# NeuroDiffGym/neurodiffeq

Hardware: NVIDIA B200
Metric: collocation-points/sec (residual+grad) (higher is better)
Workload: dtype f32

## Files before the change

experiments/tcgen05_probe/probe_wgrad.cu:

```cuda
#include <cstdio>
#include <cstdlib>
#include <cstdint>
#include <cmath>
#include <vector>
#include <cuda_runtime.h>
#include <cuda_bf16.h>

#define CK(x) do { cudaError_t e_ = (x); if (e_ != cudaSuccess) { printf("CUDA error %s at %s:%d\n", cudaGetErrorString(e_), __FILE__, __LINE__); return 2; } } while (0)

__device__ __forceinline__ uint32_t smem_u32(const void* p) { return (uint32_t)__cvta_generic_to_shared(p); }

__device__ __forceinline__ uint64_t make_desc(uint32_t saddr, uint32_t lbo_enc, uint32_t sbo_enc) {
    uint64_t d = 0;
    d |= (uint64_t)((saddr & 0x3FFFF) >> 4);
    d |= (uint64_t)(lbo_enc & 0x3FFF) << 16;
    d |= (uint64_t)(sbo_enc & 0x3FFF) << 32;
    d |= (uint64_t)1 << 46;
    d |= (uint64_t)2 << 61;
    return d;
}

constexpr int ROWS = 256, H = 64, IMG = ROWS * 128;

__global__ void __launch_bounds__(128, 1) probe_kernel(const uint8_t* __restrict__ z_img, const uint8_t* __restrict__ a_img,
// ... 41 lines not shown
            smem_u32(mbar))
        : "memory");
    asm volatile("tcgen05.fence::after_thread_sync;" ::: "memory");

    const uint32_t lane_addr = taddr + ((uint32_t)(warp * 32) << 16);
    const int tl = warp * 32 + lane;
#pragma unroll
    for (int c0 = 0; c0 < H; c0 += 16) {
        uint32_t v[16];
        asm volatile(
            "tcgen05.ld.sync.aligned.32x32b.x16.b32 {%0,%1,%2,%3,%4,%5,%6,%7,%8,%9,%10,%11,%12,%13,%14,%15}, [%16];\n"
            : "=r"(v[0]), "=r"(v[1]), "=r"(v[2]), "=r"(v[3]), "=r"(v[4]), "=r"(v[5]), "=r"(v[6]), "=r"(v[7]), "=r"(v[8]),
              "=r"(v[9]), "=r"(v[10]), "=r"(v[11]), "=r"(v[12]), "=r"(v[13]), "=r"(v[14]), "=r"(v[15])
            : "r"(lane_addr + c0));
        asm volatile("tcgen05.wait::ld.sync.aligned;" ::: "memory");
#pragma unroll
        for (int j = 0; j < 16; ++j) d_out[tl * H + c0 + j] = __uint_as_float(v[j]);
    }
    asm volatile("tcgen05.fence::before_thread_sync;" ::: "memory");
    __syncthreads();
    if (warp == 0) asm volatile("tcgen05.dealloc.cta_group::1.sync.aligned.b32 %0, 64;" ::"r"(taddr));
}

static inline size_t sw128_offset(int r, int u) {
    const int b = u * 2;
    return (size_t)(r >> 3) * 1024 + (size_t)(r & 7) * 128 + (size_t)(((b >> 4) ^ (r & 7)) << 4) + (b & 15);
}

int main(int argc, char** argv) {
    const uint32_t lbo = argc > 1 ? atoi(argv[1]) : 0, sbo = argc > 2 ? atoi(argv[2]) : 64;
    const int M = argc > 3 ? atoi(argv[3]) : 64, k_adv = argc > 4 ? atoi(argv[4]) : 2048;
    std::vector<float> Z0(ROWS * H), Z1(ROWS * H), A(ROWS * H);
    srand(3);
    for (auto& x : Z0) x = (float)(rand() % 7 - 3);
    for (auto& x : Z1) x = (float)(rand() % 5 - 2);
    for (auto& x : A) x = (float)(rand() % 7 - 3);
    std::vector<uint8_t> zi(2 * IMG, 0), ai(IMG, 0);
    for (int r = 0; r < ROWS; ++r)
        for (int u = 0; u < H; ++u) {
            *reinterpret_cast<__nv_bfloat16*>(&zi[sw128_offset(r, u)]) = __float2bfloat16(Z0[r * H + u]);
            *reinterpret_cast<__nv_bfloat16*>(&zi[IMG + sw128_offset(r, u)]) = __float2bfloat16(Z1[r * H + u]);
            *reinterpret_cast<__nv_bfloat16*>(&ai[sw128_offset(r, u)]) = __float2bfloat16(A[r * H + u]);
        }
    std::vector<double> ref(128 * H, 0.0);
    for (int m = 0; m < 128; ++m)
        for (int n = 0; n < H; ++n) {
            double s = 0;
            for (int r = 0; r < ROWS; ++r) s += (double)(m < 64 ? Z0[r * H + m] : Z1[r * H + m - 64]) * (double)A[r * H + n];
            ref[m * H + n] = s;
        }
    uint8_t *dz, *da;
    float* dd;
// ... 25 lines not shown
```

neurodiffeq_b200/csrc/pinnjet_k2tc2.cuh:

```cuda
#pragma once
#include "pinnjet_tc.cuh"

namespace pj {

constexpr int K2T_THREADS = TC_NT + 64;
#ifndef PJ_WG_FIRST
#define PJ_WG_FIRST 0
#endif

template <int N1, int N2, int WL>
__device__ __forceinline__ void act_from_record(int act, const float (&z)[1 + N1 + N2], float (&a)[1 + N1 + N2], const float* w) {
    float a0, s1, s2;
    if (act == PJ_ACT_TANH) {
        a0 = z[0];
        s1 = fmaf(-a0, a0, 1.0f);
        s2 = -2.0f * a0 * s1;
    } else {
        sincosf(z[0], &a0, &s1);
        s2 = -a0;
    }
    a[0] = a0;
#pragma unroll
    for (int f = 0; f < N1; ++f) a[1 + f] = s1 * z[1 + f];
    if constexpr (WL > 0) {
        float q = 0.0f;
#pragma unroll
        for (int d = 0; d < WL; ++d) q = fmaf(w[d] * z[1 + d], z[1 + d], q);
        a[1 + N1] = fmaf(s2, q, s1 * z[1 + N1]);
    } else {
#pragma unroll
        for (int s = 0; s < N2; ++s) a[1 + N1 + s] = fmaf(s2 * z[1 + s], z[1 + s], s1 * z[1 + N1 + s]);
// ... 15 lines not shown
    unsigned char* wimg = smem + pl.k2_ring;
    float* stage = reinterpret_cast<float*>(smem + pl.k2_zb);
    float* wlo_s = reinterpret_cast<float*>(smem + pl.k2_small);
    float* tinfo = wlo_s + sp.n_nets * PJ_MAX_NETS * TC_H;
    float* recbuf = reinterpret_cast<float*>(smem + pl.k2_ybar);
    float* sgrad = reinterpret_cast<float*>(smem + pl.k2_sgrad);
    uint64_t* wfull = reinterpret_cast<uint64_t*>(smem + pl.k2_misc);
    uint64_t* z_ready = wfull + 1;
    uint64_t* a_ready = wfull + 2;
    uint64_t* adj_done = wfull + 3;
    uint64_t* wg_done = wfull + 4;
    uint64_t* rec_full = wfull + 5;
    uint64_t* rec_empty = wfull + 6;
    uint64_t* ti_full = wfull + 7;
    uint64_t* ti_empty = wfull + 9;
    uint32_t* tmem_slot = reinterpret_cast<uint32_t*>(wfull + 11);

    const int tid = threadIdx.x, warp = tid >> 5, lane = tid & 31;
    const int n_tiles = pl.n_tiles1;
    const int my_tiles = (n_tiles > (int)blockIdx.x) ? (n_tiles - 1 - (int)blockIdx.x) / (int)gridDim.x + 1 : 0;
    float* gpart = A.gpart + (size_t)blockIdx.x * sp.n_theta;
    int n_hh = 0;
    for (int n = 0; n < sp.n_nets; ++n) n_hh += sp.net[n].n_linear - 2;
    const int tmem_cols = 64 * (1 + n_hh) <= 128 ? 128 : (64 * (1 + n_hh) <= 256 ? 256 : 512);

    pdl_launch_dependents();
    if (tid == 0) {
#ifdef PJ_TIMING
        *reinterpret_cast<unsigned long long*>(tmem_slot + 2) = clock64();
#endif
        mbar_init(wfull, 1);
        mbar_init(z_ready, TC_NCW);
        mbar_init(a_ready, TC_NCW);
        mbar_init(adj_done, 1);
        mbar_init(wg_done, 1);
        mbar_init(rec_full, 1);
        mbar_init(rec_empty, TC_NCW);
        for (int b = 0; b < 2; ++b) {
            mbar_init(&ti_full[b], 1);
            mbar_init(&ti_empty[b], TC_NCW);
        }
        fence_barrier_init();
    }
    if (warp == 0) {
        if (tmem_cols == 128)
            asm volatile("tcgen05.alloc.cta_group::1.sync.aligned.shared::cta.b32 [%0], 128;" ::"r"(smem_u32(tmem_slot)));
        else if (tmem_cols == 256)
            asm volatile("tcgen05.alloc.cta_group::1.sync.aligned.shared::cta.b32 [%0], 256;" ::"r"(smem_u32(tmem_slot)));
        else
            asm volatile("tcgen05.alloc.cta_group::1.sync.aligned.shared::cta.b32 [%0], 512;" ::"r"(smem_u32(tmem_slot)));
        asm volatile("tcgen05.relinquish_alloc_permit.cta_group::1.sync.aligned;");
    }
    for (int i = tid; i < 4 * pl.sgrad_floats; i += K2T_THREADS) sgrad[i] = 0.0f;
    if constexpr (G::CP != C)
        for (int i = tid; i < 2 * 3 * TC_AIMG / 16; i += K2T_THREADS) reinterpret_cast<uint4*>(zimg)[i] = make_uint4(0, 0, 0, 0);
    pdl_wait();
    for (int i = tid; i < sp.n_nets * PJ_MAX_NETS * TC_H; i += K2T_THREADS) {
        const int n = i / (PJ_MAX_NETS * TC_H), r = i - n * (PJ_MAX_NETS * TC_H);
        wlo_s[i] = r < sp.net[n].width[sp.net[n].n_linear] * TC_H ? __ldg(A.pack + pl.s_wlo[n] + r) : 0.0f;
    }
    for (long long i = tid; i < sp.n_theta; i += K2T_THREADS) gpart[i] = 0.0f;
    fence_proxy_async();
    tc_fence_before();
    __syncthreads();
    tc_fence_after();
    const uint32_t tmem_base = *tmem_slot;
#ifdef PJ_TIMING
    const unsigned long long t0_ = *reinterpret_cast<volatile unsigned long long*>(tmem_slot + 2);
#endif

    if (warp == TC_NCW) {
        TC_TRACE(tr, A.dbg, 250, 120, t0_, blockIdx.x == 0 && lane == 0)
        if (lane == 0) {
            if (n_hh > 0) {
                mbar_arrive_expect_tx(wfull, (uint32_t)n_hh * 3u * TC_WIMG);
                int slot = 0;
                for (int n = 0; n < sp.n_nets; ++n)
                    for (int l = 1; l < sp.net[n].n_linear - 1; ++l, ++slot)
                        tma_bulk_g2s(wimg + (size_t)slot * 3 * TC_WIMG, A.pack + pl.b_wimg[n][l], 3 * TC_WIMG, wfull);
            } else {
                mbar_arrive(wfull);
            }
        }
        mbar_wait(wfull, 0);
        constexpr uint32_t IDESC_ADJ = tc_idesc(128, TC_H, false, true), IDESC_WG = tc_idesc(64, TC_H, true, true);
        const uint64_t dz = umma_desc_sw128(smem_u32(zimg)), da = umma_desc_sw128(smem_u32(aimg));
        uint32_t phz = 0, pha = 0;
#pragma unroll 1
        for (int iter = 0; iter < my_tiles; ++iter) {
            int slot0 = 0;
#pragma unroll 1
            for (int n = 0; n < sp.n_nets; ++n) {
                const int L = sp.net[n].n_linear - 1;
#pragma unroll 1
                for (int h = L; h >= 2; --h) {
                    const int slot = slot0 + (h - 2);
                    mbar_wait(z_ready, phz);
                    phz ^= 1u;
                    tc_fence_after();
                    TC_MARK(tr, 1 | (h << 5))
                    if (lane == 0) {
                        tc_mma_split6<TC_H / 16, TC_AIMG, 32, TC_WIMG, 2048>(
                            tmem_base, dz, umma_desc_sw128(smem_u32(wimg + (size_t)slot * 3 * TC_WIMG)), IDESC_ADJ, false);
                        tc_commit(adj_done);
                    }
                    __syncwarp();
                    TC_MARK(tr, 2 | (h << 5))
                    mbar_wait(a_ready, pha);
                    pha ^= 1u;
                    tc_fence_after();
                    TC_MARK(tr, 3 | (h << 5))
                    if (lane == 0) {
                        tc_mma_split6<TC_ROWS / 16, TC_AIMG, 2048, TC_AIMG, 2048, PJ_WG_FIRST>(tmem_base + 64u + (uint32_t)slot * 64u, dz, da,
                                                                                               IDESC_WG, iter > 0);
                        tc_commit(wg_done);
                    }
                    __syncwarp();
                    TC_MARK(tr, 4 | (h << 5))
                }
                slot0 += L - 1;
            }
        }
        return;
    }

    if (warp == TC_NCW + 1) {
        uint32_t ph = 0;
        bool first = true;
        const int NW = sp.n_nets * WL, ti_rows = sp.n_yrows + NW + sp.n_coords;
        auto stage_tile_info = [&](int it) {
            if (it >= 2) mbar_wait(&ti_empty[it & 1], (uint32_t)(((it >> 1) - 1) & 1));
            const long long t = (long long)blockIdx.x + (long long)it * gridDim.x;
            float* dst = tinfo + (size_t)(it & 1) * ti_rows * TP;
            for (int e = lane; e < ti_rows * TP; e += 32) {
                const int row = e / TP, pt = e - row * TP;
                float v;
                if (row < sp.n_yrows) v = __ldg(A.seeds + t * ((long long)sp.n_yrows * TP) + e);
                else if (row < sp.n_yrows + NW) v = __ldg(A.wts + t * ((long long)NW * TP) + (e - sp.n_yrows * TP));
                else v = __ldg(A.coords[row - sp.n_yrows - NW] + min(t * TP + pt, A.N - 1));
                dst[e] = v;
            }
            __syncwarp();
            if (lane == 0) mbar_arrive(&ti_full[it & 1]);
        };
        if (my_tiles > 0) stage_tile_info(0);
#pragma unroll 1
        for (int iter = 0; iter < my_tiles; ++iter) {
            const long long tile = (long long)blockIdx.x + (long long)iter * gridDim.x;
            int lidx0 = 0;
#pragma unroll 1
            for (int n = 0; n < sp.n_nets; ++n) {
                const int L = sp.net[n].n_linear - 1;
#pragma unroll 1
                for (int h = L; h >= 1; --h) {
                    if (!first) {
                        mbar_wait(rec_empty, ph);
                        ph ^= 1u;
                    }
                    first = false;
                    if (lane == 0) {
                        mbar_arrive_expect_tx(rec_full, REC_BYTES);
                        tma_bulk_g2s(recbuf, A.zj + tile * pl.tc_rec_tile_floats + (long long)(lidx0 + h - 1) * pl.tc_rec_layer_floats,
                                     REC_BYTES, rec_full);
                    }
                    __syncwarp();
                    if (n == sp.n_nets - 1 && h == 1 && iter + 1 < my_tiles) stage_tile_info(iter + 1);
                }
                lidx0 += L;
            }
        }
        return;
    }

    const TcThread<C> th(tid);
    float* sg = sgrad + (size_t)th.q * pl.sgrad_floats;
    const bool adder = (th.pt & 1) == 0;
    const int uadd = th.ubase + (th.pt >> 1);
    uint32_t ph_adj = 0, ph_wg = 0, ph_rec = 0;
    bool wg_pending = false;
    TC_TRACE(tr, A.dbg, 0, 250, t0_, blockIdx.x == 0 && tid == 0)
    float zr[C][UG];
#ifdef PJ_DBG_REC_GLOBAL
    long long dbg_rec_off = 0;
#endif
    auto next_record = [&]() {
        mbar_wait(rec_full, ph_rec);
        ph_rec ^= 1u;
#ifdef PJ_DBG_REC_GLOBAL
        tc_load_record<C>(A.zj + dbg_rec_off + (size_t)tid * G::REC, zr);
#else
        tc_load_record_smem<C>(recbuf + (size_t)tid * G::REC, zr);
#endif
        float chk = 0.0f;
#pragma unroll
        for (int c = 0; c < C; ++c)
#pragma unroll
            for (int k = 0; k < UG; ++k) chk += zr[c][k];
        fence_proxy_async();
        __syncwarp();
        if (lane == 0 && __float_as_uint(chk) != 0xFFFFFFFFu) mbar_arrive(rec_empty);
    };

#pragma unroll 1
    for (int iter = 0; iter < my_tiles; ++iter) {
        const int NW = sp.n_nets * WL;
        const float* ti = tinfo + (size_t)(iter & 1) * (sp.n_yrows + NW + sp.n_coords) * TP + th.p;
        mbar_wait(&ti_full[iter & 1], (uint32_t)((iter >> 1) & 1));

#pragma unroll 1
        for (int n = 0; n < sp.n_nets; ++n) {
            const PjNet& net = sp.net[n];
            const int L = net.n_linear - 1;
            const int act_kind = net.act;
            const int n_out = net.width[net.n_linear];
            TC_MARK(tr, 1)
            float wq[WLN];
#pragma unroll
            for (int d = 0; d < WLN; ++d) wq[d] = WL > 0 ? ti[(sp.n_yrows + n * WL + d) * TP] : 0.0f;
            float yb_[PJ_MAX_NETS][C];
            {
                const float* sd = ti + net.yrow0 * TP;
#pragma unroll
                for (int o = 0; o < PJ_MAX_NETS; ++o)
#pragma unroll
                    for (int c = 0; c < C; ++c) yb_[o][c] = o < n_out ? sd[(o * C + c) * TP] : 0.0f;
            }
#ifdef PJ_DBG_REC_GLOBAL
            int dbg_l0 = 0;
            for (int m = 0; m < n; ++m) dbg_l0 += sp.net[m].n_linear - 1;
            dbg_rec_off = tile * pl.tc_rec_tile_floats + (long long)(dbg_l0 + L - 1) * pl.tc_rec_layer_floats;
#endif
            next_record();
            TC_MARK(tr, 2)

            float zb[C][UG];
            {
                const float* wlo = wlo_s + n * PJ_MAX_NETS * TC_H;
                float gwl[PJ_MAX_NETS][UG], gbv[UG];
#pragma unroll
                for (int k = 0; k < UG; ++k) {
                    const int u = th.ubase + k;
                    float z[C], ab[C], a[C], zbk[C];
#pragma unroll
                    for (int c = 0; c < C; ++c) {
                        z[c] = zr[c][k];
                        ab[c] = 0.0f;
                    }
#pragma unroll
                    for (int o = 0; o < PJ_MAX_NETS; ++o)
                        if (o < n_out) {
                            const float w = wlo[o * TC_H + u];
#pragma unroll
                            for (int c = 0; c < C; ++c) ab[c] = fmaf(w, yb_[o][c], ab[c]);
                        }
// ... 12 lines not shown
                {
                    const float s = tc_reduce_points<C>(gbv, th.pt);
                    if (adder) sg[pl.g_b[n][L - 1] + uadd] += s;
                }
#pragma unroll
                for (int o = 0; o < PJ_MAX_NETS; ++o)
                    if (o < n_out) {
                        const float s = tc_reduce_points<C>(gwl[o], th.pt);
                        if (adder) sg[pl.g_wl[n] + o * TC_H + uadd] += s;
                    }
                if (th.j == 0) {
#pragma unroll
                    for (int o = 0; o < PJ_MAX_NETS; ++o)
                        if (o < n_out) {
                            const float s = warp_sum(th.ug == 0 ? yb_[o][0] : 0.0f);
                            if (lane == 0) sg[pl.g_bout[n] + o] += s;
                        }
                }
            }
            TC_MARK(tr, 3)

            if (L >= 2) {
                if (wg_pending) {
                    mbar_wait(wg_done, ph_wg);
                    ph_wg ^= 1u;
                    wg_pending = false;
                }
                tc_store_rows<C>(zimg, TC_AIMG, th, zb);
                tc_publish(z_ready, th.lane);
            }
            TC_MARK(tr, 4)
#pragma unroll 1
            for (int h = L; h >= 2; --h) {
#ifdef PJ_DBG_REC_GLOBAL
                dbg_rec_off -= pl.tc_rec_layer_floats;
#endif
                next_record();
                {
                    float av[C][UG];
#pragma unroll
                    for (int k = 0; k < UG; ++k) {
                        float z[C], a[C];
#pragma unroll
                        for (int c = 0; c < C; ++c) z[c] = zr[c][k];
                        act_from_record<N1, N2, WL>(act_kind, z, a, wq);
#pragma unroll
                        for (int c = 0; c < C; ++c) av[c][k] = a[c];
                    }
                    tc_store_rows<C>(aimg, TC_AIMG, th, av);
                }
                tc_publish(a_ready, th.lane);
                TC_MARK(tr, 5 | (h << 5))

                mbar_wait(adj_done, ph_adj);
                ph_adj ^= 1u;
                tc_fence_after();
                TC_MARK(tr, 6 | (h << 5))
                float ab[C][UG];
                tc_load_owner<C>(tmem_base, stage, th, ab);
                TC_MARK(tr, 7 | (h << 5))
                float gbv[UG];
#pragma unroll
                for (int k = 0; k < UG; ++k) {
                    float z[C], abk[C], a[C], zbk[C];
#pragma unroll
                    for (int c = 0; c < C; ++c) {
                        z[c] = zr[c][k];
                        abk[c] = ab[c][k];
                    }
                    act_backward<N1, N2, WL>(act_kind, z, abk, a, zbk, wq);
#pragma unroll
                    for (int c = 0; c < C; ++c) zb[c][k] = zbk[c];
                    gbv[k] = zbk[0];
                }
                {
                    const float s = tc_reduce_points<C>(gbv, th.pt);
                    if (adder) sg[pl.g_b[n][h - 2] + uadd] += s;
                }
                TC_MARK(tr, 8 | (h << 5))
                wg_pending = true;
                if (h > 2) {
                    mbar_wait(wg_done, ph_wg);
                    ph_wg ^= 1u;
                    wg_pending = false;
                    TC_MARK(tr, 9 | (h << 5))
                    tc_store_rows<C>(zimg, TC_AIMG, th, zb);
                    tc_publish(z_ready, th.lane);
                    TC_MARK(tr, 10 | (h << 5))
                }
            }

            {
#pragma unroll
                for (int i = 0; i < PJ_MAX_COORDS; ++i)
                    if (i < net.n_in) {
                        const int ci = net.in_coord[i];
                        const float x = ti[(sp.n_yrows + NW + ci) * TP];
                        float v[UG];
#pragma unroll
                        for (int k = 0; k < UG; ++k) {
                            float s = zb[0][k] * x;
#pragma unroll
                            for (int f = 0; f < N1; ++f) s = fmaf(zb[1 + f][k], sp.dir[f][ci], s);
                            v[k] = s;
                        }
                        const float s = tc_reduce_points<C>(v, th.pt);
                        if (adder) sg[pl.g_w0[n] + uadd * net.n_in + i] += s;
                    }
            }
            TC_MARK(tr, 11)
        }
        __syncwarp();
        if (lane == 0) mbar_arrive(&ti_empty[iter & 1]);
    }
    TC_MARK(tr, 12)
    if (wg_pending) {
        mbar_wait(wg_done, ph_wg);
        ph_wg ^= 1u;
    }
    TC_MARK(tr, 14)

    tc_fence_after();
    {
        const int SG = pl.sgrad_floats;
        int slot = 0;
#pragma unroll 1
        for (int n = 0; n < sp.n_nets; ++n) {
            bar_named(9, TC_NT);
            TC_MARK(tr, 15)
            const PjNet& net = sp.net[n];
            bool shared_w = false;
            for (int m = 0; m < n; ++m) shared_w = shared_w || sp.net[m].w_off[0] == net.w_off[0];
            const int L = net.n_linear - 1;
            const int h1 = net.width[1], hL = net.width[L], n_out = net.width[net.n_linear];
            auto put = [&](long long off, int s_idx) {
                const float v = (sgrad[s_idx] + sgrad[SG + s_idx]) + (sgrad[2 * SG + s_idx] + sgrad[3 * SG + s_idx]);
                if (shared_w) gpart[off] += v; else gpart[off] = v;
            };
#pragma unroll 1
            for (int e = tid; e < h1 * net.n_in; e += TC_NT) put(net.w_off[0] + e, pl.g_w0[n] + e);
#pragma unroll 1
            for (int hl = 0; hl < L; ++hl)
#pragma unroll 1
                for (int e = tid; e < net.width[hl + 1]; e += TC_NT) put(net.b_off[hl] + e, pl.g_b[n][hl] + e);
#pragma unroll 1
            for (int e = tid; e < n_out * hL; e += TC_NT) {
                const int o = e / hL, k = e - o * hL;
                put(net.w_off[L] + e, pl.g_wl[n] + o * TC_H + k);
            }
#pragma unroll 1
            for (int e = tid; e < n_out; e += TC_NT) put(net.b_off[L] + e, pl.g_bout[n] + e);
            TC_MARK(tr, 16)
#pragma unroll 1
            for (int l = 1; l < L; ++l, ++slot) {
                const int width_j = net.width[l + 1], width_k = net.width[l];
                uint32_t v[16];
                const uint32_t addr = tmem_base + 64u + (uint32_t)slot * 64u + (uint32_t)(th.j * 16) + ((uint32_t)(th.q * 32) << 16);
                asm volatile(
                    "tcgen05.ld.sync.aligned.32x32b.x16.b32 "
                    "{%0,%1,%2,%3,%4,%5,%6,%7,%8,%9,%10,%11,%12,%13,%14,%15}, [%16];\n"
                    : "=r"(v[0]), "=r"(v[1]), "=r"(v[2]), "=r"(v[3]), "=r"(v[4]), "=r"(v[5]), "=r"(v[6]), "=r"(v[7]), "=r"(v[8]),
                      "=r"(v[9]), "=r"(v[10]), "=r"(v[11]), "=r"(v[12]), "=r"(v[13]), "=r"(v[14]), "=r"(v[15])
                    : "r"(addr));
                asm volatile("tcgen05.wait::ld.sync.aligned;" ::: "memory");
                const int jr = 16 * th.q + lane, k0 = th.j * 16;
                if (lane < 16 && jr < width_j) {
                    float* gw = gpart + net.w_off[l] + (size_t)jr * width_k + k0;
#pragma unroll
                    for (int i = 0; i < 16; ++i)
                        if (k0 + i < width_k) {
                            if (shared_w) gw[i] += __uint_as_float(v[i]); else gw[i] = __uint_as_float(v[i]);
                        }
                }
            }
        }
    }
    TC_MARK(tr, 13)
    tc_fence_before();
    bar_named(9, TC_NT);
    if (warp == 0) {
        if (tmem_cols == 128)
            asm volatile("tcgen05.dealloc.cta_group::1.sync.aligned.b32 %0, 128;" ::"r"(tmem_base));
        else if (tmem_cols == 256)
            asm volatile("tcgen05.dealloc.cta_group::1.sync.aligned.b32 %0, 256;" ::"r"(tmem_base));
        else
            asm volatile("tcgen05.dealloc.cta_group::1.sync.aligned.b32 %0, 512;" ::"r"(tmem_base));
    }
}

}
```

neurodiffeq_b200/csrc/pinnjet_tc.cuh:

```cuda
#pragma once
#include "pinnjet_common.cuh"

namespace pj {

constexpr int TC_ROWS = 128;
constexpr int TC_H = 64;
constexpr int TC_AIMG = TC_ROWS * 128;
constexpr int TC_WIMG = TC_H * 128;
constexpr int TC_WOUT = 16 * 128;
constexpr int TC_NCW = 16;
constexpr int TC_NT = TC_NCW * 32;
constexpr int TC_STAGE_STRIDE = 20;
constexpr int TC_STAGE_BYTES = TC_NCW * 32 * TC_STAGE_STRIDE * 4;

template <int C>
struct TcGeo {
    static constexpr int CP = C <= 2 ? 2 : (C <= 4 ? 4 : 8);
    static constexpr int TP = TC_ROWS / CP;
    static constexpr int PW = 32 / CP;
    static constexpr int NUG = 32 / PW;
    static constexpr int UG = 16 / NUG;
    static constexpr int REC = C * UG;
};

__device__ __forceinline__ uint64_t umma_desc_sw128(uint32_t saddr) {
    return (uint64_t)((saddr & 0x3FFFF) >> 4) | ((uint64_t)64 << 32) | ((uint64_t)1 << 46) | ((uint64_t)2 << 61);
}
__device__ __forceinline__ uint32_t sw128_off(int row, int chunk16) {
    return (uint32_t)((row >> 3) * 1024 + (row & 7) * 128 + ((chunk16 ^ (row & 7)) << 4));
}
__device__ __forceinline__ uint32_t pack_bf16x2(float lo, float hi) {
    uint32_t r;
    asm("cvt.rn.bf16x2.f32 %0, %1, %2;" : "=r"(r) : "f"(hi), "f"(lo));
    return r;
}
__device__ __forceinline__ float bf16_lo_f32(uint32_t v) { return __uint_as_float(v << 16); }
__device__ __forceinline__ float bf16_hi_f32(uint32_t v) { return __uint_as_float(v & 0xffff0000u); }

__device__ __forceinline__ void split3_bf16(float x0, float x1, uint32_t& t1, uint32_t& t2, uint32_t& t3) {
    t1 = pack_bf16x2(x0, x1);
    const float r0 = x0 - bf16_lo_f32(t1), r1 = x1 - bf16_hi_f32(t1);
    t2 = pack_bf16x2(r0, r1);
    t3 = pack_bf16x2(r0 - bf16_lo_f32(t2), r1 - bf16_hi_f32(t2));
}

__device__ __forceinline__ void bar_named(int id, int nthreads) {
    asm volatile("bar.sync %0, %1;" ::"r"(id), "r"(nthreads) : "memory");
}
__device__ __forceinline__ void tc_fence_before() { asm volatile("tcgen05.fence::before_thread_sync;" ::: "memory"); }
__device__ __forceinline__ void tc_fence_after() { asm volatile("tcgen05.fence::after_thread_sync;" ::: "memory"); }

__host__ __device__ constexpr uint32_t tc_idesc(int M, int N, bool a_mn, bool b_mn) {
    return (1u << 4) | (1u << 7) | (1u << 10) | (a_mn ? (1u << 15) : 0u) | (b_mn ? (1u << 16) : 0u) |
           ((uint32_t)(N >> 3) << 17) | ((uint32_t)(M >> 4) << 24);
}
__device__ __forceinline__ void tc_mma(uint32_t d_tmem, uint64_t da, uint64_t db, uint32_t idesc, uint32_t accumulate) {
    asm volatile(
        "{\n\t.reg .pred p;\n\tsetp.ne.b32 p, %4, 0;\n\t"
        "tcgen05.mma.cta_group::1.kind::f16 [%0], %1, %2, %3, p;\n\t}\n" ::"r"(d_tmem),
        "l"(da), "l"(db), "r"(idesc), "r"(accumulate)
        : "memory");
}
__device__ __forceinline__ void tc_commit(uint64_t* bar) {
    asm volatile("tcgen05.commit.cta_group::1.mbarrier::arrive::one.shared::cluster.b64 [%0];" ::"r"(smem_u32(bar)) : "memory");
}
template <int KSTEPS, uint32_t A_IMG, uint32_t A_KSTEP, uint32_t B_IMG, uint32_t B_KSTEP, int FIRST = 0>
__device__ __forceinline__ void tc_mma_split6(uint32_t d_tmem, uint64_t da0, uint64_t db0, uint32_t idesc, bool accumulate_first) {
#pragma unroll
    for (int pr = FIRST; pr < 6; ++pr)
#pragma unroll
        for (int k = 0; k < KSTEPS; ++k) {
            constexpr int TA[6] = {0, 2, 1, 0, 1, 0}, TB[6] = {2, 0, 1, 1, 0, 0};
            const uint64_t da = da0 + (uint64_t)((TA[pr] * A_IMG + k * A_KSTEP) >> 4);
            const uint64_t db = db0 + (uint64_t)((TB[pr] * B_IMG + k * B_KSTEP) >> 4);
            tc_mma(d_tmem, da, db, idesc, (accumulate_first || pr > FIRST || k) ? 1u : 0u);
        }
}

#ifdef PJ_TIMING
struct TcTrace {
    uint32_t* buf;
    int n, cap;
    unsigned long long t0;
    bool on;
    __device__ __forceinline__ void mark(int tag) {
        if (on && n < cap) buf[n++] = ((uint32_t)tag << 24) | (uint32_t)((clock64() - t0) & 0xFFFFFFull);
    }
};
#define TC_TRACE(name, dbg, base, cap_, t0_, on_) TcTrace name{reinterpret_cast<uint32_t*>(dbg) + (base), 0, cap_, t0_, on_};
#define TC_MARK(name, tag) name.mark(tag);
#else
#define TC_TRACE(name, dbg, base, cap_, t0_, on_)
#define TC_MARK(name, tag)
#endif

template <int C>
struct TcThread {
    using G = TcGeo<C>;
    int warp, lane, q, j, pt, ug;
// ... 29 lines not shown
    constexpr int UG = TcGeo<C>::UG;
#pragma unroll
    for (int c = 0; c < C; ++c) {
        uint32_t t1[UG / 2], t2[UG / 2], t3[UG / 2];
#pragma unroll
        for (int e = 0; e < UG / 2; ++e) split3_bf16(v[c][2 * e], v[c][2 * e + 1], t1[e], t2[e], t3[e]);
        unsigned char* dst = img + t.img_off(c);
        if constexpr (UG == 2) {
            *reinterpret_cast<uint32_t*>(dst) = t1[0];
            *reinterpret_cast<uint32_t*>(dst + img_bytes) = t2[0];
            *reinterpret_cast<uint32_t*>(dst + 2 * img_bytes) = t3[0];
        } else if constexpr (UG == 4) {
            *reinterpret_cast<uint2*>(dst) = make_uint2(t1[0], t1[1]);
            *reinterpret_cast<uint2*>(dst + img_bytes) = make_uint2(t2[0], t2[1]);
            *reinterpret_cast<uint2*>(dst + 2 * img_bytes) = make_uint2(t3[0], t3[1]);
        } else {
            *reinterpret_cast<uint4*>(dst) = make_uint4(t1[0], t1[1], t1[2], t1[3]);
            *reinterpret_cast<uint4*>(dst + img_bytes) = make_uint4(t2[0], t2[1], t2[2], t2[3]);
            *reinterpret_cast<uint4*>(dst + 2 * img_bytes) = make_uint4(t3[0], t3[1], t3[2], t3[3]);
        }
    }
}

template <int C>
__device__ __forceinline__ void tc_load_owner(uint32_t tmem_acc, float* stage, const TcThread<C>& t,
                                              float (&v)[C][TcGeo<C>::UG]) {
    using G = TcGeo<C>;
    constexpr int UG = G::UG;
    float* my_stage = stage + (size_t)t.warp * 32 * TC_STAGE_STRIDE;
    {
        uint32_t r[16];
        const uint32_t addr = tmem_acc + (uint32_t)(t.j * 16) + ((uint32_t)(t.q * 32) << 16);
        asm volatile(
            "tcgen05.ld.sync.aligned.32x32b.x16.b32 "
            "{%0,%1,%2,%3,%4,%5,%6,%7,%8,%9,%10,%11,%12,%13,%14,%15}, [%16];\n"
            : "=r"(r[0]), "=r"(r[1]), "=r"(r[2]), "=r"(r[3]), "=r"(r[4]), "=r"(r[5]), "=r"(r[6]), "=r"(r[7]), "=r"(r[8]),
              "=r"(r[9]), "=r"(r[10]), "=r"(r[11]), "=r"(r[12]), "=r"(r[13]), "=r"(r[14]), "=r"(r[15])
            : "r"(addr));
        asm volatile("tcgen05.wait::ld.sync.aligned;" ::: "memory");
        float* dst = my_stage + t.lane * TC_STAGE_STRIDE;
#pragma unroll
        for (int s = 0; s < 4; ++s)
            *reinterpret_cast<uint4*>(dst + 4 * s) = make_uint4(r[4 * s], r[4 * s + 1], r[4 * s + 2], r[4 * s + 3]);
    }
    __syncwarp();
    const float* src = my_stage + (size_t)(G::CP * t.pt) * TC_STAGE_STRIDE + t.ug * UG;
#pragma unroll
    for (int c = 0; c < C; ++c) {
        if constexpr (UG == 2) {
            const float2 x = *reinterpret_cast<const float2*>(src + c * TC_STAGE_STRIDE);
            v[c][0] = x.x;
            v[c][1] = x.y;
        } else {
#pragma unroll
            for (int s4 = 0; s4 < UG / 4; ++s4) {
                const float4 x = *reinterpret_cast<const float4*>(src + c * TC_STAGE_STRIDE + 4 * s4);
                v[c][4 * s4 + 0] = x.x;
                v[c][4 * s4 + 1] = x.y;
                v[c][4 * s4 + 2] = x.z;
                v[c][4 * s4 + 3] = x.w;
            }
        }
// ... 105 lines not shown
```

Baseline: 155.5 million.

## Stack split-bf16 MMA terms into wider N=128 tcgen05 tiles and TMA-stage tile info

For networks with few hidden layers, the six split-bf16 product terms of the adjoint and weight-gradient GEMMs are grouped into stacked M128xN128 MMAs using an LBO-strided descriptor, with the partial blocks summed when read back from tensor memory. This cuts the number of MMA instructions and makes better use of the tensor core. Tile-info staging moves from a per-lane load loop to TMA bulk copies issued by the MMA warp, prefetched ahead. Gradient zeroing is skipped when every parameter is owned. The change uses more tensor-memory columns and shared scratch, and needs an extra cross-warp reduction step before gradients are written.

```diff
diff --git a/experiments/tcgen05_probe/probe_wgrad.cu b/experiments/tcgen05_probe/probe_wgrad.cu
--- a/experiments/tcgen05_probe/probe_wgrad.cu
+++ b/experiments/tcgen05_probe/probe_wgrad.cu
@@ -87,12 +87,138 @@
     if (warp == 0) asm volatile("tcgen05.dealloc.cta_group::1.sync.aligned.b32 %0, 64;" ::"r"(taddr));
 }
 
+constexpr int TIMG = 128 * 128, WIMG = 64 * 128;
+__global__ void __launch_bounds__(128, 1) stack_kernel(const uint8_t* __restrict__ z_img, const uint8_t* __restrict__ a_img,
+                                                       const uint8_t* __restrict__ w_img, float* __restrict__ d_out) {
+    extern __shared__ __align__(1024) uint8_t smem[];
+    uint8_t* z_s = smem;
+    uint8_t* a_s = smem + 3 * TIMG;
+    uint8_t* w_s = smem + 6 * TIMG;
+    uint64_t* mbar = reinterpret_cast<uint64_t*>(smem + 6 * TIMG + 3 * WIMG);
+    uint32_t* tmem_slot = reinterpret_cast<uint32_t*>(mbar + 1);
+    const int tid = threadIdx.x, warp = tid >> 5, lane = tid & 31;
+    if (tid == 0) {
+        asm volatile("mbarrier.init.shared::cta.b64 [%0], 1;" ::"r"(smem_u32(mbar)));
+        asm volatile("fence.mbarrier_init.release.cluster;" ::: "memory");
+    }
+    if (warp == 0) {
+        asm volatile("tcgen05.alloc.cta_group::1.sync.aligned.shared::cta.b32 [%0], 512;" ::"r"(smem_u32(tmem_slot)));
+        asm volatile("tcgen05.relinquish_alloc_permit.cta_group::1.sync.aligned;");
+    }
+    for (int i = tid; i < 3 * TIMG / 16; i += 128) {
+        reinterpret_cast<uint4*>(z_s)[i] = reinterpret_cast<const uint4*>(z_img)[i];
+        reinterpret_cast<uint4*>(a_s)[i] = reinterpret_cast<const uint4*>(a_img)[i];
+    }
+    for (int i = tid; i < 3 * WIMG / 16; i += 128) reinterpret_cast<uint4*>(w_s)[i] = reinterpret_cast<const uint4*>(w_img)[i];
+    asm volatile("fence.proxy.async.shared::cta;" ::: "memory");
+    asm volatile("tcgen05.fence::before_thread_sync;" ::: "memory");
+    __syncthreads();
+    asm volatile("tcgen05.fence::after_thread_sync;" ::: "memory");
+    const uint32_t taddr = *tmem_slot;
+    if (tid == 0) {
+        auto mma = [](uint32_t d, uint64_t da, uint64_t db, uint32_t idesc, uint32_t acc) {
+            asm volatile(
+                "{\n\t.reg .pred p;\n\tsetp.ne.b32 p, %4, 0;\n\t"
+                "tcgen05.mma.cta_group::1.kind::f16 [%0], %1, %2, %3, p;\n\t}\n" ::"r"(d),
+                "l"(da), "l"(db), "r"(idesc), "r"(acc)
+                : "memory");
+        };
+        auto idesc = [](int M, int N, bool amn, bool bmn) {
+            return (1u << 4) | (1u << 7) | (1u << 10) | (amn ? 1u << 15 : 0u) | (bmn ? 1u << 16 : 0u) | ((uint32_t)(N >> 3) << 17) |
+                   ((uint32_t)(M >> 4) << 24);
+        };
+        const uint32_t za = smem_u32(z_s), aa = smem_u32(a_s), wa = smem_u32(w_s);
+        for (int k = 0; k < 8; ++k)
+            mma(taddr, make_desc(za + k * 2048, TIMG >> 4, 64), make_desc(aa + k * 2048, TIMG >> 4, 64), idesc(128, 128, true, true), k);
+        for (int k = 0; k < 8; ++k)
+            mma(taddr + 128, make_desc(za + k * 2048, 0, 64), make_desc(aa + 2 * TIMG + k * 2048, 0, 64), idesc(64, 64, true, true), k);
+        for (int k = 0; k < 8; ++k)
+            mma(taddr + 128, make_desc(za + 2 * TIMG + k * 2048, 0, 64), make_desc(aa + k * 2048, 0, 64), idesc(64, 64, true, true), 1);
+        for (int k = 0; k < 4; ++k)
+            mma(taddr + 192, make_desc(za + k * 32, 0, 64), make_desc(wa + k * 2048, WIMG >> 4, 64), idesc(128, 128, false, true), k);
+        asm volatile("tcgen05.commit.cta_group::1.mbarrier::arrive::one.shared::cluster.b64 [%0];" ::"r"(smem_u32(mbar)) : "memory");
+    }
+    asm volatile(
+        "{\n.reg .pred P1;\nLAB_WAIT2:\nmbarrier.try_wait.parity.shared::cta.b64 P1, [%0], 0;\n@P1 bra DONE2;\nbra LAB_WAIT2;\nDONE2:\n}\n" ::"r"(
+            smem_u32(mbar))
+        : "memory");
+    asm volatile("tcgen05.fence::after_thread_sync;" ::: "memory");
+    const uint32_t lane_addr = taddr + ((uint32_t)(warp * 32) << 16);
+    const int tl = warp * 32 + lane;
+    for (int c0 = 0; c0 < 320; c0 += 16) {
+        uint32_t v[16];
+        asm volatile(
+            "tcgen05.ld.sync.aligned.32x32b.x16.b32 {%0,%1,%2,%3,%4,%5,%6,%7,%8,%9,%10,%11,%12,%13,%14,%15}, [%16];\n"
+            : "=r"(v[0]), "=r"(v[1]), "=r"(v[2]), "=r"(v[3]), "=r"(v[4]), "=r"(v[5]), "=r"(v[6]), "=r"(v[7]), "=r"(v[8]),
+              "=r"(v[9]), "=r"(v[10]), "=r"(v[11]), "=r"(v[12]), "=r"(v[13]), "=r"(v[14]), "=r"(v[15])
+            : "r"(lane_addr + c0));
+        asm volatile("tcgen05.wait::ld.sync.aligned;" ::: "memory");
+        for (int j = 0; j < 16; ++j) d_out[tl * 320 + c0 + j] = __uint_as_float(v[j]);
+    }
+    asm volatile("tcgen05.fence::before_thread_sync;" ::: "memory");
+    __syncthreads();
+    if (warp == 0) asm volatile("tcgen05.dealloc.cta_group::1.sync.aligned.b32 %0, 512;" ::"r"(taddr));
+}
+
 static inline size_t sw128_offset(int r, int u) {
     const int b = u * 2;
     return (size_t)(r >> 3) * 1024 + (size_t)(r & 7) * 128 + (size_t)(((b >> 4) ^ (r & 7)) << 4) + (b & 15);
 }
 
+static int run_stack() {
+    const int R = 128;
+    std::vector<float> Z[3], A[3], W[3];
+    srand(5);
+    for (int t = 0; t < 3; ++t) {
+        Z[t].resize(R * H); A[t].resize(R * H); W[t].resize(H * H);
+        for (auto& x : Z[t]) x = (float)(rand() % 7 - 3);
+        for (auto& x : A[t]) x = (float)(rand() % 5 - 2);
+        for (auto& x : W[t]) x = (float)(rand() % 7 - 3);
+    }
+    std::vector<uint8_t> zi(3 * TIMG, 0), ai(3 * TIMG, 0), wi(3 * WIMG, 0);
+    for (int t = 0; t < 3; ++t)
+        for (int r = 0; r < R; ++r)
+            for (int u = 0; u < H; ++u) {
+                *reinterpret_cast<__nv_bfloat16*>(&zi[t * TIMG + sw128_offset(r, u)]) = __float2bfloat16(Z[t][r * H + u]);
+                *reinterpret_cast<__nv_bfloat16*>(&ai[t * TIMG + sw128_offset(r, u)]) = __float2bfloat16(A[t][r * H + u]);
+                if (r < H) *reinterpret_cast<__nv_bfloat16*>(&wi[t * WIMG + sw128_offset(r, u)]) = __float2bfloat16(W[t][r * H + u]);
+            }
+    uint8_t *dz, *da, *dw;
+    float* dd;
+    const int smem_bytes = 6 * TIMG + 3 * WIMG + 64;
+    CK(cudaMalloc(&dz, 3 * TIMG)); CK(cudaMalloc(&da, 3 * TIMG)); CK(cudaMalloc(&dw, 3 * WIMG)); CK(cudaMalloc(&dd, 128 * 320 * 4));
+    CK(cudaMemcpy(dz, zi.data(), zi.size(), cudaMemcpyHostToDevice));
+    CK(cudaMemcpy(da, ai.data(), ai.size(), cudaMemcpyHostToDevice));
+    CK(cudaMemcpy(dw, wi.data(), wi.size(), cudaMemcpyHostToDevice));
+    CK(cudaMemset(dd, 0xff, 128 * 320 * 4));
+    CK(cudaFuncSetAttribute(stack_kernel, cudaFuncAttributeMaxDynamicSharedMemorySize, smem_bytes));
+    stack_kernel<<<1, 128, smem_bytes>>>(dz, da, dw, dd);
+    CK(cudaGetLastError());
+    CK(cudaDeviceSynchronize());
+    std::vector<float> out(128 * 320);
+    CK(cudaMemcpy(out.data(), dd, out.size() * 4, cudaMemcpyDeviceToHost));
+    double e0 = 0, e1 = 0, e2 = 0;
+    for (int m = 0; m < 128; ++m)
+        for (int n = 0; n < 128; ++n) {
+            double s = 0, s2 = 0;
+            for (int r = 0; r < R; ++r) s += (double)Z[m / 64][r * H + m % 64] * A[n / 64][r * H + n % 64];
+            for (int j = 0; j < H; ++j) s2 += (double)Z[0][m * H + j] * W[n / 64][j * H + n % 64];
+            e0 = fmax(e0, fabs(out[m * 320 + n] - s));
+            e2 = fmax(e2, fabs(out[m * 320 + 192 + n] - s2));
+        }
+    for (int j = 0; j < 64; ++j)
+        for (int n = 0; n < 64; ++n) {
+            double s = 0;
+            for (int r = 0; r < R; ++r) s += (double)Z[0][r * H + j] * A[2][r * H + n] + (double)Z[2][r * H + j] * A[0][r * H + n];
+            e1 = fmax(e1, fabs(out[((j % 16) + 32 * (j / 16)) * 320 + 128 + n] - s));
+        }
+    printf("stack probe: WG M128xN128 MN-major LBO 16 KB max|err| %.3g   WG M64 (13 + 31) max|err| %.3g   "
+           "ADJ M128xN128 B MN-major LBO 8 KB max|err| %.3g\n", e0, e1, e2);
+    return (e0 == 0.0 && e1 == 0.0 && e2 == 0.0) ? 0 : 1;
+}
+
 int main(int argc, char** argv) {
+    if (argc > 1 && argv[1][0] == 's') return run_stack();
     const uint32_t lbo = argc > 1 ? atoi(argv[1]) : 0, sbo = argc > 2 ? atoi(argv[2]) : 64;
     const int M = argc > 3 ? atoi(argv[3]) : 64, k_adv = argc > 4 ? atoi(argv[4]) : 2048;
     std::vector<float> Z0(ROWS * H), Z1(ROWS * H), A(ROWS * H);
diff --git a/neurodiffeq_b200/csrc/pinnjet_k2tc2.cuh b/neurodiffeq_b200/csrc/pinnjet_k2tc2.cuh
--- a/neurodiffeq_b200/csrc/pinnjet_k2tc2.cuh
+++ b/neurodiffeq_b200/csrc/pinnjet_k2tc2.cuh
@@ -4,9 +4,7 @@
 namespace pj {
 
 constexpr int K2T_THREADS = TC_NT + 64;
-#ifndef PJ_WG_FIRST
-#define PJ_WG_FIRST 0
-#endif
+constexpr int K2T_WG_ROW = 68;
 
 template <int N1, int N2, int WL>
 __device__ __forceinline__ void act_from_record(int act, const float (&z)[1 + N1 + N2], float (&a)[1 + N1 + N2], const float* w) {
@@ -68,7 +66,10 @@
     float* gpart = A.gpart + (size_t)blockIdx.x * sp.n_theta;
     int n_hh = 0;
     for (int n = 0; n < sp.n_nets; ++n) n_hh += sp.net[n].n_linear - 2;
-    const int tmem_cols = 64 * (1 + n_hh) <= 128 ? 128 : (64 * (1 + n_hh) <= 256 ? 256 : 512);
+    const bool stacked = n_hh <= 2;
+    const int adj_cols = stacked ? 128 : 64, wg_cols = stacked ? 192 : 64;
+    const int need_cols = adj_cols + wg_cols * n_hh;
+    const int tmem_cols = need_cols <= 128 ? 128 : (need_cols <= 256 ? 256 : 512);
 
     pdl_launch_dependents();
     if (tid == 0) {
@@ -105,7 +106,18 @@
         const int n = i / (PJ_MAX_NETS * TC_H), r = i - n * (PJ_MAX_NETS * TC_H);
         wlo_s[i] = r < sp.net[n].width[sp.net[n].n_linear] * TC_H ? __ldg(A.pack + pl.s_wlo[n] + r) : 0.0f;
     }
-    for (long long i = tid; i < sp.n_theta; i += K2T_THREADS) gpart[i] = 0.0f;
+    {
+        long long owned = 0;
+        for (int n = 0; n < sp.n_nets; ++n) {
+            bool shared_w = false;
+            for (int m = 0; m < n; ++m) shared_w = shared_w || sp.net[m].w_off[0] == sp.net[n].w_off[0];
+            if (!shared_w)
+                for (int l = 0; l < sp.net[n].n_linear; ++l)
+                    owned += (long long)sp.net[n].width[l + 1] * (sp.net[n].width[l] + 1);
+        }
+        if (owned != sp.n_theta)
+            for (long long i = tid; i < sp.n_theta; i += K2T_THREADS) gpart[i] = 0.0f;
+    }
     fence_proxy_async();
     tc_fence_before();
     __syncthreads();
@@ -115,6 +127,7 @@
     const unsigned long long t0_ = *reinterpret_cast<volatile unsigned long long*>(tmem_slot + 2);
 #endif
 
+    const int NW = sp.n_nets * WL, ti_rows = sp.n_yrows + NW + sp.n_coords;
     if (warp == TC_NCW) {
         TC_TRACE(tr, A.dbg, 250, 120, t0_, blockIdx.x == 0 && lane == 0)
         if (lane == 0) {
@@ -128,12 +141,39 @@
                 mbar_arrive(wfull);
             }
         }
+        auto stage_tile_info = [&](int it) {
+            if (it >= 2) mbar_wait(&ti_empty[it & 1], (uint32_t)(((it >> 1) - 1) & 1));
+            const long long t = (long long)blockIdx.x + (long long)it * gridDim.x;
+            float* dst = tinfo + (size_t)(it & 1) * ti_rows * TP;
+            bool bulk_xy = (t + 1) * TP <= A.N;
+            for (int i = 0; i < sp.n_coords; ++i) bulk_xy = bulk_xy && (reinterpret_cast<uintptr_t>(A.coords[i]) & 15) == 0;
+            if (!bulk_xy) {
+                for (int e = lane; e < sp.n_coords * TP; e += 32) {
+                    const int row = e / TP, pt = e - row * TP;
+                    dst[(sp.n_yrows + NW) * TP + e] = __ldg(A.coords[row] + min(t * TP + pt, A.N - 1));
+                }
+                __syncwarp();
+            }
+            if (lane == 0) {
+                const uint32_t sbytes = (uint32_t)(sp.n_yrows * TP * 4), wbytes = (uint32_t)(NW * TP * 4);
+                mbar_arrive_expect_tx(&ti_full[it & 1], sbytes + wbytes + (bulk_xy ? (uint32_t)(sp.n_coords * TP * 4) : 0u));
+                tma_bulk_g2s(dst, A.seeds + t * ((long long)sp.n_yrows * TP), sbytes, &ti_full[it & 1]);
+                if (NW > 0) tma_bulk_g2s(dst + sp.n_yrows * TP, A.wts + t * ((long long)NW * TP), wbytes, &ti_full[it & 1]);
+                if (bulk_xy)
+                    for (int i = 0; i < sp.n_coords; ++i)
+                        tma_bulk_g2s(dst + (sp.n_yrows + NW + i) * TP, A.coords[i] + t * TP, TP * 4, &ti_full[it & 1]);
+            }
+            __syncwarp();
+        };
+        if (my_tiles > 0) stage_tile_info(0);
+        if (my_tiles > 1) stage_tile_info(1);
         mbar_wait(wfull, 0);
         constexpr uint32_t IDESC_ADJ = tc_idesc(128, TC_H, false, true), IDESC_WG = tc_idesc(64, TC_H, true, true);
         const uint64_t dz = umma_desc_sw128(smem_u32(zimg)), da = umma_desc_sw128(smem_u32(aimg));
         uint32_t phz = 0, pha = 0;
 #pragma unroll 1
         for (int iter = 0; iter < my_tiles; ++iter) {
+            if (iter >= 1 && iter + 1 < my_tiles) stage_tile_info(iter + 1);
             int slot0 = 0;
 #pragma unroll 1
             for (int n = 0; n < sp.n_nets; ++n) {
@@ -141,13 +181,17 @@
 #pragma unroll 1
                 for (int h = L; h >= 2; --h) {
                     const int slot = slot0 + (h - 2);
+                    const uint32_t wsl = smem_u32(wimg + (size_t)slot * 3 * TC_WIMG);
+                    const uint32_t d_wg = tmem_base + (uint32_t)(adj_cols + slot * wg_cols);
                     mbar_wait(z_ready, phz);
                     phz ^= 1u;
                     tc_fence_after();
                     TC_MARK(tr, 1 | (h << 5))
                     if (lane == 0) {
-                        tc_mma_split6<TC_H / 16, TC_AIMG, 32, TC_WIMG, 2048>(
-                            tmem_base, dz, umma_desc_sw128(smem_u32(wimg + (size_t)slot * 3 * TC_WIMG)), IDESC_ADJ, false);
+                        if (stacked)
+                            tc_mma_adj_stacked(tmem_base, dz, wsl);
+                        else
+                            tc_mma_split6<TC_H / 16, TC_AIMG, 32, TC_WIMG, 2048>(tmem_base, dz, umma_desc_sw128(wsl), IDESC_ADJ, false);
                         tc_commit(adj_done);
                     }
                     __syncwarp();
@@ -157,8 +201,10 @@
                     tc_fence_after();
                     TC_MARK(tr, 3 | (h << 5))
                     if (lane == 0) {
-                        tc_mma_split6<TC_ROWS / 16, TC_AIMG, 2048, TC_AIMG, 2048, PJ_WG_FIRST>(tmem_base + 64u + (uint32_t)slot * 64u, dz, da,
-                                                                                               IDESC_WG, iter > 0);
+                        if (stacked)
+                            tc_mma_wg_stacked(d_wg, smem_u32(zimg), smem_u32(aimg), iter > 0);
+                        else
+                            tc_mma_split6<TC_ROWS / 16, TC_AIMG, 2048, TC_AIMG, 2048>(d_wg, dz, da, IDESC_WG, iter > 0);
                         tc_commit(wg_done);
                     }
                     __syncwarp();
@@ -173,23 +219,6 @@
     if (warp == TC_NCW + 1) {
         uint32_t ph = 0;
         bool first = true;
-        const int NW = sp.n_nets * WL, ti_rows = sp.n_yrows + NW + sp.n_coords;
-        auto stage_tile_info = [&](int it) {
-            if (it >= 2) mbar_wait(&ti_empty[it & 1], (uint32_t)(((it >> 1) - 1) & 1));
-            const long long t = (long long)blockIdx.x + (long long)it * gridDim.x;
-            float* dst = tinfo + (size_t)(it & 1) * ti_rows * TP;
-            for (int e = lane; e < ti_rows * TP; e += 32) {
-                const int row = e / TP, pt = e - row * TP;
-                float v;
-                if (row < sp.n_yrows) v = __ldg(A.seeds + t * ((long long)sp.n_yrows * TP) + e);
-                else if (row < sp.n_yrows + NW) v = __ldg(A.wts + t * ((long long)NW * TP) + (e - sp.n_yrows * TP));
-                else v = __ldg(A.coords[row - sp.n_yrows - NW] + min(t * TP + pt, A.N - 1));
-                dst[e] = v;
-            }
-            __syncwarp();
-            if (lane == 0) mbar_arrive(&ti_full[it & 1]);
-        };
-        if (my_tiles > 0) stage_tile_info(0);
 #pragma unroll 1
         for (int iter = 0; iter < my_tiles; ++iter) {
             const long long tile = (long long)blockIdx.x + (long long)iter * gridDim.x;
@@ -210,7 +239,6 @@
                                      REC_BYTES, rec_full);
                     }
                     __syncwarp();
-                    if (n == sp.n_nets - 1 && h == 1 && iter + 1 < my_tiles) stage_tile_info(iter + 1);
                 }
                 lidx0 += L;
             }
@@ -222,21 +250,15 @@
     float* sg = sgrad + (size_t)th.q * pl.sgrad_floats;
     const bool adder = (th.pt & 1) == 0;
     const int uadd = th.ubase + (th.pt >> 1);
-    uint32_t ph_adj = 0, ph_wg = 0, ph_rec = 0;
+    uint32_t ph_adj = 0;
     bool wg_pending = false;
     TC_TRACE(tr, A.dbg, 0, 250, t0_, blockIdx.x == 0 && tid == 0)
+    uint32_t ph_rec = 0;
     float zr[C][UG];
-#ifdef PJ_DBG_REC_GLOBAL
-    long long dbg_rec_off = 0;
-#endif
     auto next_record = [&]() {
         mbar_wait(rec_full, ph_rec);
         ph_rec ^= 1u;
-#ifdef PJ_DBG_REC_GLOBAL
-        tc_load_record<C>(A.zj + dbg_rec_off + (size_t)tid * G::REC, zr);
-#else
         tc_load_record_smem<C>(recbuf + (size_t)tid * G::REC, zr);
-#endif
         float chk = 0.0f;
 #pragma unroll
         for (int c = 0; c < C; ++c)
@@ -249,8 +271,7 @@
 
 #pragma unroll 1
     for (int iter = 0; iter < my_tiles; ++iter) {
-        const int NW = sp.n_nets * WL;
-        const float* ti = tinfo + (size_t)(iter & 1) * (sp.n_yrows + NW + sp.n_coords) * TP + th.p;
+        const float* ti = tinfo + (size_t)(iter & 1) * ti_rows * TP + th.p;
         mbar_wait(&ti_full[iter & 1], (uint32_t)((iter >> 1) & 1));
 
 #pragma unroll 1
@@ -271,11 +292,6 @@
 #pragma unroll
                     for (int c = 0; c < C; ++c) yb_[o][c] = o < n_out ? sd[(o * C + c) * TP] : 0.0f;
             }
-#ifdef PJ_DBG_REC_GLOBAL
-            int dbg_l0 = 0;
-            for (int m = 0; m < n; ++m) dbg_l0 += sp.net[m].n_linear - 1;
-            dbg_rec_off = tile * pl.tc_rec_tile_floats + (long long)(dbg_l0 + L - 1) * pl.tc_rec_layer_floats;
-#endif
             next_record();
             TC_MARK(tr, 2)
 
@@ -334,8 +350,7 @@
 
             if (L >= 2) {
                 if (wg_pending) {
-                    mbar_wait(wg_done, ph_wg);
-                    ph_wg ^= 1u;
+                    mbar_wait(wg_done, ph_adj ^ 1u);
                     wg_pending = false;
                 }
                 tc_store_rows<C>(zimg, TC_AIMG, th, zb);
@@ -344,9 +359,6 @@
             TC_MARK(tr, 4)
 #pragma unroll 1
             for (int h = L; h >= 2; --h) {
-#ifdef PJ_DBG_REC_GLOBAL
-                dbg_rec_off -= pl.tc_rec_layer_floats;
-#endif
                 next_record();
                 {
                     float av[C][UG];
@@ -369,7 +381,7 @@
                 tc_fence_after();
                 TC_MARK(tr, 6 | (h << 5))
                 float ab[C][UG];
-                tc_load_owner<C>(tmem_base, stage, th, ab);
+                tc_load_owner<C>(tmem_base, stage, th, ab, stacked);
                 TC_MARK(tr, 7 | (h << 5))
                 float gbv[UG];
 #pragma unroll
@@ -392,8 +404,7 @@
                 TC_MARK(tr, 8 | (h << 5))
                 wg_pending = true;
                 if (h > 2) {
-                    mbar_wait(wg_done, ph_wg);
-                    ph_wg ^= 1u;
+                    mbar_wait(wg_done, ph_adj ^ 1u);
                     wg_pending = false;
                     TC_MARK(tr, 9 | (h << 5))
                     tc_store_rows<C>(zimg, TC_AIMG, th, zb);
@@ -422,14 +433,12 @@
             }
             TC_MARK(tr, 11)
         }
+        fence_proxy_async();
         __syncwarp();
         if (lane == 0) mbar_arrive(&ti_empty[iter & 1]);
     }
     TC_MARK(tr, 12)
-    if (wg_pending) {
-        mbar_wait(wg_done, ph_wg);
-        ph_wg ^= 1u;
-    }
+    if (wg_pending) mbar_wait(wg_done, ph_adj ^ 1u);
     TC_MARK(tr, 14)
 
     tc_fence_after();
@@ -463,27 +472,43 @@
 #pragma unroll 1
             for (int e = tid; e < n_out; e += TC_NT) put(net.b_off[L] + e, pl.g_bout[n] + e);
             TC_MARK(tr, 16)
+            float* wsum = reinterpret_cast<float*>(zimg);
 #pragma unroll 1
             for (int l = 1; l < L; ++l, ++slot) {
                 const int width_j = net.width[l + 1], width_k = net.width[l];
+                const uint32_t acc = tmem_base + (uint32_t)(adj_cols + slot * wg_cols) + (uint32_t)(th.j * 16) + ((uint32_t)(th.q * 32) << 16);
                 uint32_t v[16];
-                const uint32_t addr = tmem_base + 64u + (uint32_t)slot * 64u + (uint32_t)(th.j * 16) + ((uint32_t)(th.q * 32) << 16);
-                asm volatile(
-                    "tcgen05.ld.sync.aligned.32x32b.x16.b32 "
-                    "{%0,%1,%2,%3,%4,%5,%6,%7,%8,%9,%10,%11,%12,%13,%14,%15}, [%16];\n"
-                    : "=r"(v[0]), "=r"(v[1]), "=r"(v[2]), "=r"(v[3]), "=r"(v[4]), "=r"(v[5]), "=r"(v[6]), "=r"(v[7]), "=r"(v[8]),
-                      "=r"(v[9]), "=r"(v[10]), "=r"(v[11]), "=r"(v[12]), "=r"(v[13]), "=r"(v[14]), "=r"(v[15])
-                    : "r"(addr));
-                asm volatile("tcgen05.wait::ld.sync.aligned;" ::: "memory");
-                const int jr = 16 * th.q + lane, k0 = th.j * 16;
-                if (lane < 16 && jr < width_j) {
-                    float* gw = gpart + net.w_off[l] + (size_t)jr * width_k + k0;
-#pragma unroll
-                    for (int i = 0; i < 16; ++i)
-                        if (k0 + i < width_k) {
-                            if (shared_w) gw[i] += __uint_as_float(v[i]); else gw[i] = __uint_as_float(v[i]);
-                        }
-                }
+                if (stacked) {
+                    uint32_t h[16];
+                    tmem_ld16(acc, v);
+                    tmem_ld16(acc + 64u, h);
+                    tmem_ld_wait();
+                    float* dst = wsum + ((th.q >> 1) * 64 + (th.q & 1) * 32 + lane) * K2T_WG_ROW + th.j * 16;
+#pragma unroll
+                    for (int s4 = 0; s4 < 4; ++s4)
+                        *reinterpret_cast<float4*>(dst + 4 * s4) = make_float4(
+                            __uint_as_float(v[4 * s4]) + __uint_as_float(h[4 * s4]), __uint_as_float(v[4 * s4 + 1]) + __uint_as_float(h[4 * s4 + 1]),
+                            __uint_as_float(v[4 * s4 + 2]) + __uint_as_float(h[4 * s4 + 2]), __uint_as_float(v[4 * s4 + 3]) + __uint_as_float(h[4 * s4 + 3]));
+                }
+                tmem_ld16(acc + (stacked ? 128u : 0u), v);
+                tmem_ld_wait();
+                if (lane < 16) {
+                    float* dst = wsum + (128 + 16 * th.q + lane) * K2T_WG_ROW + th.j * 16;
+#pragma unroll
+                    for (int s4 = 0; s4 < 4; ++s4)
+                        *reinterpret_cast<float4*>(dst + 4 * s4) = make_float4(__uint_as_float(v[4 * s4]), __uint_as_float(v[4 * s4 + 1]),
+                                                                              __uint_as_float(v[4 * s4 + 2]), __uint_as_float(v[4 * s4 + 3]));
+                }
+                bar_named(9, TC_NT);
+#pragma unroll 1
+                for (int e = tid; e < width_j * width_k; e += TC_NT) {
+                    const int jr = e / width_k, k = e - jr * width_k;
+                    float w = wsum[(128 + jr) * K2T_WG_ROW + k];
+                    if (stacked) w = (w + wsum[(64 + jr) * K2T_WG_ROW + k]) + wsum[jr * K2T_WG_ROW + k];
+                    float* gw = gpart + net.w_off[l] + e;
+                    if (shared_w) *gw += w; else *gw = w;
+                }
+                bar_named(9, TC_NT);
             }
         }
     }
diff --git a/neurodiffeq_b200/csrc/pinnjet_tc.cuh b/neurodiffeq_b200/csrc/pinnjet_tc.cuh
--- a/neurodiffeq_b200/csrc/pinnjet_tc.cuh
+++ b/neurodiffeq_b200/csrc/pinnjet_tc.cuh
@@ -26,6 +26,9 @@
 __device__ __forceinline__ uint64_t umma_desc_sw128(uint32_t saddr) {
     return (uint64_t)((saddr & 0x3FFFF) >> 4) | ((uint64_t)64 << 32) | ((uint64_t)1 << 46) | ((uint64_t)2 << 61);
 }
+__device__ __forceinline__ uint64_t umma_desc_sw128_lbo(uint32_t saddr, uint32_t lbo) {
+    return umma_desc_sw128(saddr) | ((uint64_t)(lbo >> 4) << 16);
+}
 __device__ __forceinline__ uint32_t sw128_off(int row, int chunk16) {
     return (uint32_t)((row >> 3) * 1024 + (row & 7) * 128 + ((chunk16 ^ (row & 7)) << 4));
 }
@@ -64,17 +67,43 @@
 __device__ __forceinline__ void tc_commit(uint64_t* bar) {
     asm volatile("tcgen05.commit.cta_group::1.mbarrier::arrive::one.shared::cluster.b64 [%0];" ::"r"(smem_u32(bar)) : "memory");
 }
-template <int KSTEPS, uint32_t A_IMG, uint32_t A_KSTEP, uint32_t B_IMG, uint32_t B_KSTEP, int FIRST = 0>
+template <int KSTEPS, uint32_t A_IMG, uint32_t A_KSTEP, uint32_t B_IMG, uint32_t B_KSTEP>
 __device__ __forceinline__ void tc_mma_split6(uint32_t d_tmem, uint64_t da0, uint64_t db0, uint32_t idesc, bool accumulate_first) {
 #pragma unroll
-    for (int pr = FIRST; pr < 6; ++pr)
+    for (int pr = 0; pr < 6; ++pr)
 #pragma unroll
         for (int k = 0; k < KSTEPS; ++k) {
             constexpr int TA[6] = {0, 2, 1, 0, 1, 0}, TB[6] = {2, 0, 1, 1, 0, 0};
             const uint64_t da = da0 + (uint64_t)((TA[pr] * A_IMG + k * A_KSTEP) >> 4);
             const uint64_t db = db0 + (uint64_t)((TB[pr] * B_IMG + k * B_KSTEP) >> 4);
-            tc_mma(d_tmem, da, db, idesc, (accumulate_first || pr > FIRST || k) ? 1u : 0u);
-        }
+            tc_mma(d_tmem, da, db, idesc, (accumulate_first || pr || k) ? 1u : 0u);
+        }
+}
+
+__device__ __forceinline__ void tc_mma_adj_stacked(uint32_t d_tmem, uint64_t dz, uint32_t w) {
+    constexpr uint32_t ID64 = tc_idesc(128, 64, false, true), ID128 = tc_idesc(128, 128, false, true);
+    const uint64_t dw = umma_desc_sw128(w), dw2 = umma_desc_sw128_lbo(w, TC_WIMG);
+#pragma unroll
+    for (int k = 0; k < 4; ++k) tc_mma(d_tmem, dz + ((k * 32) >> 4), dw + ((2 * TC_WIMG + k * 2048) >> 4), ID64, k ? 1u : 0u);
+#pragma unroll
+    for (int k = 0; k < 4; ++k) tc_mma(d_tmem + 64, dz + ((2 * TC_AIMG + k * 32) >> 4), dw + ((k * 2048) >> 4), ID64, k ? 1u : 0u);
+#pragma unroll
+    for (int t = 1; t >= 0; --t)
+#pragma unroll
+        for (int k = 0; k < 4; ++k) tc_mma(d_tmem, dz + ((t * TC_AIMG + k * 32) >> 4), dw2 + ((k * 2048) >> 4), ID128, 1u);
+}
+__device__ __forceinline__ void tc_mma_wg_stacked(uint32_t d_tmem, uint32_t z, uint32_t a, bool accumulate_first) {
+    constexpr uint32_t ID64 = tc_idesc(64, 64, true, true), ID128 = tc_idesc(128, 128, true, true);
+    const uint64_t dz = umma_desc_sw128(z), da = umma_desc_sw128(a);
+    const uint64_t dz2 = umma_desc_sw128_lbo(z, TC_AIMG), da2 = umma_desc_sw128_lbo(a, TC_AIMG);
+#pragma unroll
+    for (int k = 0; k < 8; ++k)
+        tc_mma(d_tmem + 128, dz + ((k * 2048) >> 4), da + ((2 * TC_AIMG + k * 2048) >> 4), ID64, (accumulate_first || k) ? 1u : 0u);
+#pragma unroll
+    for (int k = 0; k < 8; ++k) tc_mma(d_tmem + 128, dz + ((2 * TC_AIMG + k * 2048) >> 4), da + ((k * 2048) >> 4), ID64, 1u);
+#pragma unroll
+    for (int k = 0; k < 8; ++k)
+        tc_mma(d_tmem, dz2 + ((k * 2048) >> 4), da2 + ((k * 2048) >> 4), ID128, (accumulate_first || k) ? 1u : 0u);
 }
 
 #ifdef PJ_TIMING
@@ -150,9 +179,19 @@
     }
 }
 
+__device__ __forceinline__ void tmem_ld16(uint32_t addr, uint32_t (&v)[16]) {
+    asm volatile(
+        "tcgen05.ld.sync.aligned.32x32b.x16.b32 "
+        "{%0,%1,%2,%3,%4,%5,%6,%7,%8,%9,%10,%11,%12,%13,%14,%15}, [%16];\n"
+        : "=r"(v[0]), "=r"(v[1]), "=r"(v[2]), "=r"(v[3]), "=r"(v[4]), "=r"(v[5]), "=r"(v[6]), "=r"(v[7]), "=r"(v[8]),
+          "=r"(v[9]), "=r"(v[10]), "=r"(v[11]), "=r"(v[12]), "=r"(v[13]), "=r"(v[14]), "=r"(v[15])
+        : "r"(addr));
+}
+__device__ __forceinline__ void tmem_ld_wait() { asm volatile("tcgen05.wait::ld.sync.aligned;" ::: "memory"); }
+
 template <int C>
 __device__ __forceinline__ void tc_load_owner(uint32_t tmem_acc, float* stage, const TcThread<C>& t,
-                                              float (&v)[C][TcGeo<C>::UG]) {
+                                              float (&v)[C][TcGeo<C>::UG], bool add_block1 = false) {
     using G = TcGeo<C>;
     constexpr int UG = G::UG;
     float* my_stage = stage + (size_t)t.warp * 32 * TC_STAGE_STRIDE;
@@ -165,7 +204,20 @@
             : "=r"(r[0]), "=r"(r[1]), "=r"(r[2]), "=r"(r[3]), "=r"(r[4]), "=r"(r[5]), "=r"(r[6]), "=r"(r[7]), "=r"(r[8]),
               "=r"(r[9]), "=r"(r[10]), "=r"(r[11]), "=r"(r[12]), "=r"(r[13]), "=r"(r[14]), "=r"(r[15])
             : "r"(addr));
-        asm volatile("tcgen05.wait::ld.sync.aligned;" ::: "memory");
+        if (add_block1) {
+            uint32_t h[16];
+            asm volatile(
+                "tcgen05.ld.sync.aligned.32x32b.x16.b32 "
+                "{%0,%1,%2,%3,%4,%5,%6,%7,%8,%9,%10,%11,%12,%13,%14,%15}, [%16];\n"
+                : "=r"(h[0]), "=r"(h[1]), "=r"(h[2]), "=r"(h[3]), "=r"(h[4]), "=r"(h[5]), "=r"(h[6]), "=r"(h[7]), "=r"(h[8]),
+                  "=r"(h[9]), "=r"(h[10]), "=r"(h[11]), "=r"(h[12]), "=r"(h[13]), "=r"(h[14]), "=r"(h[15])
+                : "r"(addr + 64u));
+            asm volatile("tcgen05.wait::ld.sync.aligned;" ::: "memory");
+#pragma unroll
+            for (int i = 0; i < 16; ++i) r[i] = __float_as_uint(__uint_as_float(r[i]) + __uint_as_float(h[i]));
+        } else {
+            asm volatile("tcgen05.wait::ld.sync.aligned;" ::: "memory");
+        }
         float* dst = my_stage + t.lane * TC_STAGE_STRIDE;
 #pragma unroll
         for (int s = 0; s < 4; ++s)
```

Result: faster. 161.8 million (median of 6 runs) (+4.1%).
